# mwhitehill/Tacotron-2

Hardware: AMD Instinct MI355X
Metric: mel-frames/sec (decoder) + audio-samples/sec (WaveNet) @1/2/4/8 MI355X (higher is better)
Workload: dtype f32; 1 GPU; configs[1]: Tacotron-2 encoder+decoder+Postnet inference, batch=32x200-char synthetic, T_out=1000, 1 batch per GPU; global_batch=32, chars=200, t_out=1000, decoded_steps=1000, ref_frames=400, parallelism=utterance-batch sharding x1

## Files before the change

tacotron-2_amd/csrc/common.h:

```cpp
#pragma once
#include <hip/hip_runtime.h>

#include <cstdint>
#include <cstdio>
#include <cstdlib>
#include <map>
#include <stdexcept>
#include <string>
#include <vector>

#include "../../include/tt2.h"

namespace tt2 {

struct Error : std::runtime_error {
  int status;
  Error(int s, const std::string& m) : std::runtime_error(m), status(s) {}
};

void set_last_error(const std::string& msg);

#define TT2_HIP(call)                                                                      \
  do {                                                                                     \
    hipError_t e_ = (call);                                                                \
// ... 102 lines not shown

void put_tensor(WeightMap& wm, const char* name, const float* host, const int64_t* shape, int ndim);
const HostTensor& need(const WeightMap& wm, const std::string& name, std::vector<int64_t> shape);

typedef float f32x4 __attribute__((ext_vector_type(4)));

__host__ __device__ inline int af_idx(int m, int k) {
  const int s = k >> 2, kk = k & 3, h = m >> 4, i = m & 15;
  return ((((s >> 2) * 2 + h) * 64 + (kk * 16 + i)) << 2) + (s & 3);
}
__host__ __device__ inline int wf_idx(int k, int j) {
  const int s = k >> 2, kk = k & 3;
  return ((((s >> 2) * 64) + (kk * 16 + j)) << 2) + (s & 3);
}

constexpr float KG_SB = 1024.f, KG_UNSCALE = 1.f / 1024.f, KG_BMAX = 63.9f;
typedef _Float16 kg_f16x4 __attribute__((ext_vector_type(4)));
typedef unsigned u32x4 __attribute__((ext_vector_type(4)));
__host__ __device__ inline void kg_split1(float v, _Float16& h, _Float16& l) {
  h = (_Float16)v;
  l = (_Float16)(v - (float)h);
}
__host__ __device__ inline void kg_split(const f32x4& v, kg_f16x4& h, kg_f16x4& l) {
#pragma unroll
  for (int e = 0; e < 4; ++e) {
    _Float16 x, y;
    kg_split1(v[e], x, y);
    h[e] = x;
    l[e] = y;
  }
}
struct alignas(16) kg_pk {
  kg_f16x4 h, l;
};
__host__ __device__ inline kg_pk kg_pack(const f32x4& v) {
  kg_pk p;
  kg_split(v, p.h, p.l);
  return p;
}
__host__ __device__ inline kg_pk kg_pk_bits(const u32x4& w) { return __builtin_bit_cast(kg_pk, w); }
__host__ __device__ inline u32x4 kg_bits(const kg_pk& p) { return __builtin_bit_cast(u32x4, p); }
__device__ __forceinline__ kg_pk kg_ld(const float* base, int i4) {
  return kg_pk_bits(reinterpret_cast<const u32x4*>(base)[i4]);
}
__device__ __forceinline__ void kg_mfma_x3_pre(const kg_pk& a0, const kg_pk& a1, const kg_pk& bw, f32x4& c0,
                                               f32x4& c1) {
  c0 = __builtin_amdgcn_mfma_f32_16x16x16f16(a0.l, bw.h, c0, 0, 0, 0);
  c1 = __builtin_amdgcn_mfma_f32_16x16x16f16(a1.l, bw.h, c1, 0, 0, 0);
  c0 = __builtin_amdgcn_mfma_f32_16x16x16f16(a0.h, bw.l, c0, 0, 0, 0);
  c1 = __builtin_amdgcn_mfma_f32_16x16x16f16(a1.h, bw.l, c1, 0, 0, 0);
  c0 = __builtin_amdgcn_mfma_f32_16x16x16f16(a0.h, bw.h, c0, 0, 0, 0);
  c1 = __builtin_amdgcn_mfma_f32_16x16x16f16(a1.h, bw.h, c1, 0, 0, 0);
}
__device__ __forceinline__ void kg_mfma_x3(const f32x4& a0, const f32x4& a1, const f32x4& bw, f32x4& c0,
                                           f32x4& c1) {
  kg_f16x4 a0h, a0l, a1h, a1l, bh, bl;
  kg_split(a0, a0h, a0l);
  kg_split(a1, a1h, a1l);
  kg_split(bw, bh, bl);
  c0 = __builtin_amdgcn_mfma_f32_16x16x16f16(a0l, bh, c0, 0, 0, 0);
  c1 = __builtin_amdgcn_mfma_f32_16x16x16f16(a1l, bh, c1, 0, 0, 0);
  c0 = __builtin_amdgcn_mfma_f32_16x16x16f16(a0h, bl, c0, 0, 0, 0);
  c1 = __builtin_amdgcn_mfma_f32_16x16x16f16(a1h, bl, c1, 0, 0, 0);
  c0 = __builtin_amdgcn_mfma_f32_16x16x16f16(a0h, bh, c0, 0, 0, 0);
  c1 = __builtin_amdgcn_mfma_f32_16x16x16f16(a1h, bh, c1, 0, 0, 0);
}

__device__ __forceinline__ void skinny_mfma(const float* __restrict__ X, const float* __restrict__ Wt,
                                            int sg0, int sg1, f32x4& acc0, f32x4& acc1, int lane) {
  const f32x4* Xv = reinterpret_cast<const f32x4*>(X);
  const f32x4* Wv = reinterpret_cast<const f32x4*>(Wt);
#pragma unroll 4
  for (int sg = sg0; sg < sg1; ++sg) {
    const f32x4 a0 = Xv[(sg * 2 + 0) * 64 + lane];
    const f32x4 a1 = Xv[(sg * 2 + 1) * 64 + lane];
    const f32x4 b = Wv[sg * 64 + lane];
#pragma unroll
    for (int j = 0; j < 4; ++j) {
      acc0 = __builtin_amdgcn_mfma_f32_16x16x4f32(a0[j], b[j], acc0, 0, 0, 0);
      acc1 = __builtin_amdgcn_mfma_f32_16x16x4f32(a1[j], b[j], acc1, 0, 0, 0);
    }
  }
}

template <int NPW>
__device__ __forceinline__ void skinny_mfma_all(const float* __restrict__ X, const float* __restrict__ Wt,
                                                int sg0, f32x4& acc0, f32x4& acc1, int lane) {
  const f32x4* Xv = reinterpret_cast<const f32x4*>(X);
  const f32x4* Wv = reinterpret_cast<const f32x4*>(Wt);
  f32x4 a0[NPW], a1[NPW], b[NPW];
#pragma unroll
  for (int j = 0; j < NPW; ++j) {
    b[j] = Wv[(sg0 + j) * 64 + lane];
    a0[j] = Xv[((sg0 + j) * 2 + 0) * 64 + lane];
    a1[j] = Xv[((sg0 + j) * 2 + 1) * 64 + lane];
  }
  __builtin_amdgcn_sched_barrier(0);
#pragma unroll
  for (int j = 0; j < NPW; ++j)
#pragma unroll
    for (int e = 0; e < 4; ++e) {
      acc0 = __builtin_amdgcn_mfma_f32_16x16x4f32(a0[j][e], b[j][e], acc0, 0, 0, 0);
      acc1 = __builtin_amdgcn_mfma_f32_16x16x4f32(a1[j][e], b[j][e], acc1, 0, 0, 0);
    }
}

// ... 131 lines not shown
```

tacotron-2_amd/csrc/decode_persist.hip:

```cpp
#include "decode_persist.h"

namespace tt2 {

typedef unsigned u32x2 __attribute__((ext_vector_type(2)));

typedef __attribute__((address_space(1))) float pd_gf32;
typedef __attribute__((address_space(1))) unsigned pd_gu32;
typedef __attribute__((address_space(1))) int pd_gi32;
typedef __attribute__((address_space(1))) unsigned long long pd_gu64;
#define PD_RLX __ATOMIC_RELAXED, __HIP_MEMORY_SCOPE_AGENT

#ifndef PD_TAG_H1
#define PD_TAG_H1 0
#endif
constexpr long long PD_TIMEOUT = 200000000LL;
constexpr int PD_LDS_FLOATS = 16384 * 2 + 4096 + 512 * 5 + 288 + 256 * 2 + 32 + 16 + 16 + 16 + 512;

__device__ __forceinline__ float pd_ld(const float* p) {
  return __hip_atomic_load((pd_gf32*)const_cast<float*>(p), PD_RLX);
}
__device__ __forceinline__ void pd_st(float* p, float v) { __hip_atomic_store((pd_gf32*)p, v, PD_RLX); }
__device__ __forceinline__ u32x4 pd_ld4(const float* base, int i4) {
  const auto r = __builtin_amdgcn_make_buffer_rsrc(const_cast<float*>(base), (short)0, 0x7fffffff, 0x00020000);
  return __builtin_amdgcn_raw_buffer_load_b128(r, i4 * 16, 0, 16);
}
__device__ __forceinline__ f32x4 pd_ld4f(const float* base, int i4) { return __builtin_bit_cast(f32x4, pd_ld4(base, i4)); }
__device__ __forceinline__ u32x2 pd_ld2(const float* base, int i2) {
  const auto r = __builtin_amdgcn_make_buffer_rsrc(const_cast<float*>(base), (short)0, 0x7fffffff, 0x00020000);
  return __builtin_amdgcn_raw_buffer_load_b64(r, i2 * 8, 0, 16);
}

template <class F>
__device__ __forceinline__ bool pd_spin(const PdArgs& a, int ph, int lane, F cond) {
  long long t0 = 0;
  for (unsigned spin = 0;; ++spin) {
    if (__all(cond())) return true;
    if ((spin & 63) == 0) {
      const long long now = __builtin_amdgcn_s_memrealtime();
      if (spin == 0) {
        t0 = now;
      } else if (__hip_atomic_load((pd_gi32*)(a.ctl + 2), PD_RLX) != 0 || now - t0 > PD_TIMEOUT) {
        if (lane == 0) __hip_atomic_store((pd_gi32*)(a.ctl + 2), 1 + ph, PD_RLX);
        return false;
      }
    }
    for (int z = 0; z < a.poll_sleep; ++z) __builtin_amdgcn_s_sleep(1);
  }
}

__device__ __forceinline__ unsigned pd_flag(const unsigned* f) {
  return __hip_atomic_load((pd_gu32*)const_cast<unsigned*>(f), PD_RLX);
}

__device__ __forceinline__ bool pd_poll(const PdArgs& a, int ph, int base, int stride, int n, unsigned need, int shift,
                                        int lane) {
  const unsigned* f = a.flags + ph * PD_NB + base;
  return pd_spin(a, ph, lane, [&] { return lane >= n || (pd_flag(f + lane * stride) >> shift) >= need; });
}

__device__ __forceinline__ bool pd_poll_all(const PdArgs& a, int ph, int nprod, unsigned need, int shift, int lane,
                                            bool sweep_first) {
  const int g = blockIdx.x, x = g >> 3, s = g & 7;
  const unsigned* f = a.flags + ph * PD_NB + 32 * s;
  unsigned* f2 = a.flags2 + ph * PD_NB + 8 * x;
  if (sweep_first) {
    const unsigned* fa = a.flags + ph * PD_NB;
    bool ok = true;
#pragma unroll
    for (int i = 0; i < 4; ++i) {
      const int pidx = lane + 64 * i;
      ok = ok && (pidx >= nprod || (pd_flag(fa + pidx) >> shift) >= need);
    }
    if (__all(ok)) {
      if (lane == 0) __hip_atomic_store((pd_gu32*)(f2 + s), need, PD_RLX);
      return true;
    }
  }
  if (!pd_spin(a, ph, lane, [&] { return lane >= 32 || 32 * s + lane >= nprod || (pd_flag(f + lane) >> shift) >= need; }))
    return false;
  if (lane == 0) __hip_atomic_store((pd_gu32*)(f2 + s), need, PD_RLX);
  return pd_spin(a, ph, lane, [&] { return lane >= 8 || pd_flag(f2 + lane) >= need; });
}

__device__ __forceinline__ bool pd_poll_rep(const PdArgs& a, int ph, int r, int base, unsigned need, int lane,
                                            int n = 32) {
  const unsigned* f = a.rflags + (r * PD_NREP + (blockIdx.x & (PD_NREP - 1))) * PD_NB + base;
  return pd_spin(a, ph, lane, [&] { return lane >= n || pd_flag(f + lane) >= need; });
}

template <class F>
__device__ __forceinline__ bool pd_block_wait(int* slot, F poll) {
  if (threadIdx.x < 64) {
    const bool ok = poll();
    if (threadIdx.x == 0) *slot = ok;
  }
  __syncthreads();
  return *slot != 0;
}

__device__ __forceinline__ void pd_putw(unsigned long long* g, unsigned tag, unsigned w) {
  __hip_atomic_store((pd_gu64*)g, ((unsigned long long)tag << 32) | w, PD_RLX);
}
// ... 118 lines not shown

__device__ __forceinline__ void pd_hint(const PdArgs& a, int ph, unsigned val, int tid) {
  __syncthreads();
  if (tid == 0) __hip_atomic_store((pd_gu32*)(a.flags + ph * PD_NB + blockIdx.x), val, PD_RLX);
}
__device__ __forceinline__ void pd_hint_rep(const PdArgs& a, int r, unsigned val, int tid) {
  __syncthreads();
  if (tid < PD_NREP) __hip_atomic_store((pd_gu32*)(a.rflags + (r * PD_NREP + tid) * PD_NB + blockIdx.x), val, PD_RLX);
}

__device__ __forceinline__ void pd_publish_rep(const PdArgs& a, int r, unsigned val, int tid) {
  asm volatile("s_waitcnt vmcnt(0)" ::: "memory");
  __syncthreads();
  if (tid < PD_NREP) __hip_atomic_store((pd_gu32*)(a.rflags + (r * PD_NREP + tid) * PD_NB + blockIdx.x), val, PD_RLX);
}

__device__ __forceinline__ void put_partials(const f32x4& acc0, const f32x4& acc1, float* red, int w, int lane) {
#pragma unroll
  for (int r = 0; r < 4; ++r) {
    const int n = lane & 15, m = (lane >> 4) * 4 + r;
    red[w * 512 + m * 16 + n] = acc0[r];
    red[w * 512 + (m + 16) * 16 + n] = acc1[r];
  }
}
template <int NW>
__device__ __forceinline__ float sum_partials(const float* red, int idx) {
  float v = red[idx];
#pragma unroll
  for (int ww = 1; ww < NW; ++ww) v += red[ww * 512 + idx];
  return v;
}

__device__ __forceinline__ void tail_bar(int* ctr, unsigned& gen, int lane) {
  gen += 4;
  asm volatile("s_waitcnt lgkmcnt(0)" ::: "memory");
  if (lane == 0) __hip_atomic_fetch_add(ctr, 1, __ATOMIC_RELEASE, __HIP_MEMORY_SCOPE_WORKGROUP);
  while ((unsigned)__hip_atomic_load(ctr, __ATOMIC_ACQUIRE, __HIP_MEMORY_SCOPE_WORKGROUP) < gen)
    __builtin_amdgcn_s_sleep(0);
}

#define PD_STAMP(i)                                                                   \
  do {                                                                                \
    if (stp && tid == 0) stp[g * 32 + (i)] = __builtin_amdgcn_s_memrealtime();        \
  } while (0)

template <bool EMT, int TM, bool FL>
__global__ __launch_bounds__(PD_NT) void k_decode_persist(PdArgs a) {
  static_assert(TM == PD_TMAX || (TM == PD_TMAX_LONG && !EMT), "k_decode_persist geometry");
  static_assert(!FL || (!EMT && TM == PD_TMAX), "floor instance: the Tacotron decoder only");
  const auto mm = [](const u32x4& x0, const u32x4& x1, const kg_pk& bw, f32x4& c0, f32x4& c1) {
    if constexpr (FL) asm volatile("" ::"v"(x0), "v"(x1), "v"(kg_bits(bw)));
    else kg_mfma_x3_pre(pd_unx(x0), pd_unx(x1), bw, c0, c1);
  };
  const auto mmo = [](const u32x4& x0, const u32x4& x1, const kg_pk& bw, f32x4& c0, f32x4& c1) {
    if constexpr (FL) asm volatile("" ::"v"(x0), "v"(x1), "v"(kg_bits(bw)));
    else kg_mfma_x3_pre(kg_pk_bits(x0), kg_pk_bits(x1), bw, c0, c1);
  };
  const auto mmg = [](const u32x4& g0, const u32x4& g1, const kg_pk& bw, f32x4& c0, f32x4& c1) {
    if constexpr (FL) asm volatile("" ::"v"(g0), "v"(g1), "v"(kg_bits(bw)));
    else kg_mfma_x3_pre(pd_ung(g0), pd_ung(g1), bw, c0, c1);
  };
  const auto mmf = [](const f32x4& a0, const f32x4& a1, const kg_pk& bw, f32x4& c0, f32x4& c1) {
    kg_mfma_x3_pre(kg_pack(a0), kg_pack(a1), bw, c0, c1);
  };
  constexpr int NI = TM / 128;
  constexpr int NWE = TM / 64;
  constexpr int CWN = TM == PD_TMAX ? 288 : 544;
  extern __shared__ __attribute__((aligned(16))) float sm[];
  float* const sW1h = sm;
  float* const sW2h = sm + 16384;
  float* const red = sm + 32768;
  float* const G = red + 4096;
  float* const RG1 = G + 512;
  float* const RG2 = RG1 + 512;
  float* const RGc = RG2 + 512;
  float* const PPh = RGc + 512;
  float* const cw = PPh + 512;
  float* const al = TM == PD_TMAX ? cw + 288 : red + 2048;
  float* const x1 = cw + 544;
  float* const ssa = x1 + 256;
  float* const qv = ssa + 32;
  float* const sc = qv + 16;
  int* const si = reinterpret_cast<int*>(sc + 16);
  const int g = blockIdx.x, tid_ = threadIdx.x;
  const int b = (g & 7) * 4 + ((g >> 3) & 3), j = g >> 5;
  const bool rowv = b < a.B;
  constexpr int NTL = EMT ? PD_NTILE + PD_ENT : PD_NTILE;
  const bool isproj = g < NTL * PD_KSP;
  const int pn = g % NTL, pks = g / NTL;
  const bool isq = EMT && isproj && pn >= PD_NTILE;
  const int K1S = EMT ? a.K1 : PD_P + PD_E2;
  const int T = a.T_in;
  const int sib0 = (b >> 2) + 8 * (b & 3);
  long long* const stp0 = a.stamps;

  const int tid = tid_, lane = tid & 63, w = tid >> 6;
  const int em = (tid >> 2) & 31, eu = tid & 3;
  kg_pk w1p[2], w2i[8];
  {
    const float* L1 = a.l1_w + (long)g * K1S * 16;
    const float* L2 = a.l2_w + (long)g * PD_H * 16;
#pragma unroll
    for (int i = 0; i < 2; ++i) w1p[i] = kg_ld(L1, (2 * w + i) * 64 + lane);
#pragma unroll
    for (int i = 0; i < 8; ++i) w2i[i] = kg_ld(L2, (8 * w + i) * 64 + lane);
    const f32x4* L1h = reinterpret_cast<const f32x4*>(a.l1_wh + (long)g * PD_H * 16);
    const f32x4* L2h = reinterpret_cast<const f32x4*>(a.l2_wh + (long)g * PD_H * 16);
    f32x4* d1 = reinterpret_cast<f32x4*>(sW1h);
    f32x4* d2 = reinterpret_cast<f32x4*>(sW2h);
    for (int e = tid; e < PD_H * 4; e += PD_NT) {
      d1[e] = L1h[e];
      d2[e] = L2h[e];
    }
  }
  const f32x4 zero4 = {0.f, 0.f, 0.f, 0.f};
  const kg_pk zeropk = kg_pk_bits(u32x4{0u, 0u, 0u, 0u});
  kg_pk wpc = zeropk;
  if (isproj && w < 4 && !isq) wpc = kg_ld(a.proj_w + (long)pn * (PD_H + PD_E2) * 16, (PD_H / 16 + 4 * pks + w) * 64 + lane);
  const float* const WPH = a.proj_w + (long)pn * (PD_H + PD_E2) * 16 + (8 * pks) * 64 * 4;
  kg_pk w1c[4];
  {
    const float* W1C = a.l1_w + (long)g * K1S * 16 + (PD_P / 16 + 4 * w) * 64 * 4;
#pragma unroll
    for (int i = 0; i < 4; ++i) w1c[i] = kg_ld(W1C, i * 64 + lane);
  }
  kg_pk w1e = zeropk, wdf = zeropk;
  if constexpr (EMT) {
    if (w < a.e_XW / 16)
      w1e = kg_ld(a.l1_w + (long)g * K1S * 16, ((PD_P + PD_E2) / 16 + w) * 64 + lane);
    if (a.e_dense && isq && w < a.e_KC / 128)
      wdf = kg_ld(a.e_wd + (long)(pn - PD_NTILE) * a.e_KC * 16, (pks * (a.e_KC / 128) + w) * 64 + lane);
  }
  f32x4* const swl = reinterpret_cast<f32x4*>(si + 16);
  if (tid < 128) swl[tid] = reinterpret_cast<const f32x4*>(a.loc_cw + (long)j * PD_KLP * 16)[tid];
  float* const cst = RG1;
  const int u0 = pd_unit(g, 0);
  if (tid < 128) {
#pragma unroll
    for (int q = 0; q < 4; ++q) {
      const int u = pd_unit(g, eu);
      const int col = (u >> 2) * 16 + 4 * q + (u & 3);
      cst[q * 128 + tid] = a.l1_b[col] + (EMT && a.e_spk1 ? a.e_spk1[(long)em * 4 * PD_H + col] : 0.f);
      cst[(4 + q) * 128 + tid] = a.l2_b[col];
      cst[(8 + q) * 128 + tid] = a.GS[(long)em * 4 * PD_H + col];
    }
  }
  float c1 = 0.f, c2 = 0.f;
  const int len = rowv ? a.lengths[b] : 0;
  const float va_k = a.va[16 * j + (lane & 15)];
  const float b2p = a.pre_b2[32 * j + (tid & 31)];
  for (int e = tid; e < CWN; e += PD_NT) cw[e] = 0.f;
  if (tid < TM) al[tid] = 0.f;
  if (tid < 32) ssa[tid] = 0.f;
  if (tid == 0) {
    si[0] = 0;
    si[4] = 0;
    si[8] = 0;
    sc[2] = 0.f;
  }
  f32x4 vals[8];
  {
    const f32x4* V = reinterpret_cast<const f32x4*>(a.valuesT + ((long)(rowv ? b : 0) * PD_E2 + 64 * j + (tid & 63)) * TM +
                                                    32 * (tid >> 6));
#pragma unroll
    for (int i = 0; i < 8; ++i) vals[i] = V[i];
  }
  f32x4 loc[NI];
#pragma unroll
  for (int i = 0; i < NI; ++i) loc[i] = zero4;
  f32x4 accC0 = zero4, accC1 = zero4;
  if constexpr (EMT) {
    const float* XE = a.EMTx + 32 * PD_EQ;
    mmf(pd_ld4f(XE, (w * 2) * 64 + lane), pd_ld4f(XE, (w * 2 + 1) * 64 + lane), w1e, accC0, accC1);
  }
  f32x4 q1a = zero4, q1b = zero4, q2a = zero4, q2b = zero4;
  const long BP = (long)a.B * PD_P;

// ... 13 lines not shown
  auto prenet_ops = [&](float k1, float k2, int tid) {
    PrenetOps o;
    o.keep1 = k1;
    o.keep2 = k2;
    const f32x4* W2 = reinterpret_cast<const f32x4*>(a.pre_w2t + (long)(32 * j + (tid & 31)) * PD_P + 16 * (tid >> 5));
#pragma unroll
    for (int i = 0; i < 4; ++i) o.w2p[i] = W2[i];
    return o;
  };
  auto prenet = [&](const PrenetOps& o, auto pre1, int par, unsigned tag, int tid) {
    if (tid >= 256) {
      const int pos = tid - 256;
      const int col = 16 * (pos >> 4) + ((pos >> 2) & 3) + 4 * (pos & 3);
      x1[col] = rowv ? (fmaxf(pre1(pos), 0.f) / 0.5f) * o.keep1 : 0.f;
      if (pos < 32) red[3072 + pos] = o.keep2;
    }
    __syncthreads();
    {
      const int k16 = tid >> 5;
      float s = 0.f;
#pragma unroll
      for (int i = 0; i < 16; ++i)
        if (!FL || i == 0) s += x1[16 * k16 + i] * o.w2p[i >> 2][i & 3];
      s += __shfl_xor(s, 32);
      if ((tid & 63) < 32) red[(tid >> 6) * 32 + (tid & 31)] = s;
    }
    __syncthreads();
    if (tid < 32) {
      float v = 0.f;
#pragma unroll
      for (int ww = 0; ww < 8; ++ww) v += red[ww * 32 + tid];
      const int n = 32 * j + tid;
      const float out = rowv ? (fmaxf(v + b2p, 0.f) / 0.5f) * red[3072 + tid] : 0.f;
      pd_putw(a.PREg + par * 32 * PD_P + af_idx(b, n), tag, pd_split1(out));
    }
  };

  auto rec_half = [&](int ph, const float* X, unsigned tb, const float* Wl, int h, f32x4& Qa, f32x4& Qb, int w,
                      int lane, bool check, bool pin) {
    u32x4 xv[8];
    const auto ix = [&](int i) { return ((8 * w + 4 * h + (i >> 1)) * 2 + (i & 1)) * 64 + lane; };
    if (check) {
      if (!pd_take4<8>(a, ph, X, ix, tb, xv, [] { return true; })) si[8] = 1;
    } else {
#pragma unroll
      for (int i = 0; i < 8; ++i) xv[i] = pd_ld4(X, ix(i));
      if (pin) __builtin_amdgcn_sched_barrier(0);
    }
    if (h == 0) {
      Qa = a.zo * Qa;
      Qb = a.zo * Qb;
    }
#pragma unroll
    for (int i = 0; i < 4; ++i) {
      const int sg = 8 * w + 4 * h + i;
      if (!PD_TAG_H1 && ph == PD_F_H1) mmo(xv[2 * i], xv[2 * i + 1], kg_ld(Wl, sg * 64 + lane), Qa, Qb);
      else mm(xv[2 * i], xv[2 * i + 1], kg_ld(Wl, sg * 64 + lane), Qa, Qb);
    }
  };
  __syncthreads();
  {
    float k1, k2;
    prenet_keep(0, tid, k1, k2);
    prenet(prenet_ops(k1, k2, tid), [&](int pos) { return a.pre_b1[pos]; }, 0, 1u << 1, tid);
  }
  if (tid == 0) si[1] = 0;
  __syncthreads();

  for (int t = 0; t < a.max_iters; ++t) {
    const unsigned tg = t + 1;
    const int p = t & 1;
    const unsigned tb = pd_tb(t), tbp = pd_tb(t - 1);
    long long* const stp = (stp0 && t == a.stamp_step) ? stp0 : nullptr;
    int tid = tid_, lane, w, em, eu;
    asm volatile("" : "+v"(tid));
    lane = tid & 63;
    w = tid >> 6;
    em = (tid >> 2) & 31;
    eu = tid & 3;
    PD_STAMP(0);
    if constexpr (!EMT) {
      if (stp && tid == 0) stp[g * 32 + 31] = __builtin_amdgcn_s_getreg(0x1814) & 15;
    }
    float keep1n, keep2n;
    prenet_keep(t + 1, tid, keep1n, keep2n);
    u32x4 a0[2], a1[2];
    {
      const auto rp = __builtin_amdgcn_make_buffer_rsrc(a.PREg + p * 32 * PD_P, (short)0, 0x7fffffff, 0x00020000);
      unsigned sb[2] = {0u, 0u};
      long long t0 = 0;
      for (unsigned spin = 0;; ++spin) {
        bool ok = true;
#pragma unroll
        for (int i = 0; i < 2; ++i)
#pragma unroll
          for (int h = 0; h < 2; ++h) {
            const int fo = (((2 * w + i) * 2 + h) * 64 + lane) * 4;
            const auto q0 = __builtin_amdgcn_raw_buffer_load_b128(rp, fo * 8, 0, 16);
            const auto q1 = __builtin_amdgcn_raw_buffer_load_b128(rp, fo * 8 + 16, 0, 16);
            const u32x4 v = {q0[0], q0[2], q1[0], q1[2]};
            ok = ok && (q0[1] >> 1) == tg && (q0[3] >> 1) == tg && (q1[1] >> 1) == tg && (q1[3] >> 1) == tg;
            if (h == 0) a0[i] = v;
            else a1[i] = v;
            if (i == 0) sb[h] = q0[1] & 1u;
          }
        if (__all(ok)) break;
        if ((spin & 31) == 0) {
          const long long now = __builtin_amdgcn_s_memrealtime();
          if (spin == 0) {
            t0 = now;
          } else if (__hip_atomic_load((pd_gi32*)(a.ctl + 2), PD_RLX) != 0 || now - t0 > PD_TIMEOUT) {
            if (lane == 0) {
              __hip_atomic_store((pd_gi32*)(a.ctl + 2), 1 + PD_F_PRE, PD_RLX);
              atomicMax(si + 1, 2);
            }
            break;
          }
        }
        for (int z = 0; z < a.poll_sleep; ++z) __builtin_amdgcn_s_sleep(1);
      }
      if (t > 0 && w == 0) {
        int dn;
        if (a.T_lim > 0) {
          dn = t >= a.T_lim;
        } else {
          const int r0 = lane & 15;
          const bool v0 = lane < 16 && r0 < a.B, v1 = lane < 16 && r0 + 16 < a.B;
          const unsigned long long f0 = __ballot(v0 && sb[0]), f1 = __ballot(v1 && sb[1]);
          const unsigned long long m0 = __ballot(v0), m1 = __ballot(v1);
          dn = a.stop_at_any == 2 ? 0 : (f0 == m0 && f1 == m1);
        }
        if (lane == 0 && dn) atomicMax(si + 1, 1);
      }
    }
    PD_STAMP(1);
    {
      f32x4 s0 = accC0 + a.one_m_zo * q1a, s1 = accC1 + a.one_m_zo * q1b;
#pragma unroll
      for (int i = 0; i < 2; ++i) mmg(a0[i], a1[i], w1p[i], s0, s1);
      PD_STAMP(18);
      put_partials(s0, s1, red, w, lane);
      __syncthreads();
      PD_STAMP(19);
    }
    if (si[1]) {
      if (si[1] == 1 && g == 0 && tid == 0) {
        a.ctl[1] = t;
        a.ctl[0] = 1;
      }
      return;
    }
    if (tid < 128) {
      float z[4];
#pragma unroll
      for (int q = 0; q < 4; ++q) {
        const int idx = em * 16 + 4 * q + eu;
        z[q] = (sum_partials<8>(red, idx) * KG_UNSCALE + ssa[em] * cst[(8 + q) * 128 + tid]) + cst[q * 128 + tid];
      }
      const float cn = sigm_fast(z[2] + 1.0f) * c1 + sigm_fast(z[0]) * tanh_rcp(z[1]);
      const float hn = sigm_fast(z[3]) * tanh_rcp(cn);
      c1 = a.one_m_zo * cn + a.zo * c1;
      pd_st_h4(a.H1x + p * 32 * PD_H, em, u0, hn, lane, PD_TAG_H1 ? tb : ~0u);
    }
    if constexpr (PD_TAG_H1) pd_hint_rep(a, 0, tg, tid);
    else pd_publish_rep(a, 0, tg, tid);
    PD_STAMP(2);
    if (t > 0) rec_half(PD_F_H2, a.H2x + (p ^ 1) * 32 * PD_H, tbp, sW2h, 1, q2a, q2b, w, lane, false, true);
    PD_STAMP(3);
    if constexpr (!PD_TAG_H1)
      if (!pd_poll_rep(a, PD_F_H1, 0, 32 * w, tg, lane)) si[8] = 1;
    PD_STAMP(4);
    {
      const float* X = a.H1x + p * 32 * PD_H;
      f32x4 s0 = a.one_m_zo * q2a, s1 = a.one_m_zo * q2b;
#pragma unroll
      for (int h = 0; h < 2; ++h) {
        u32x4 xv[8];
        const auto ix = [&](int i) { return ((8 * w + 4 * h + (i >> 1)) * 2 + (i & 1)) * 64 + lane; };
        if constexpr (PD_TAG_H1 == 0) {
#pragma unroll
          for (int i = 0; i < 8; ++i) xv[i] = pd_ld4(X, ix(i));
          __builtin_amdgcn_sched_barrier(0);
        } else if constexpr (PD_TAG_H1 == 1) {
          if (!pd_take4<8>(a, PD_F_H1, X, ix, tb, xv, [&] { return pd_poll_rep(a, PD_F_H1, 0, 32 * w, tg, lane); }))
            si[8] = 1;
        } else {
          if (!pd_take4<8>(a, PD_F_H1, X, ix, tb, xv, [] { return true; })) si[8] = 1;
        }
#pragma unroll
        for (int i = 0; i < 4; ++i) {
          if constexpr (PD_TAG_H1) mm(xv[2 * i], xv[2 * i + 1], w2i[4 * h + i], s0, s1);
          else mmo(xv[2 * i], xv[2 * i + 1], w2i[4 * h + i], s0, s1);
        }
      }
      PD_STAMP(16);
      put_partials(s0, s1, red, w, lane);
      __syncthreads();
      PD_STAMP(17);
      if (si[8]) return;
    }
    if (tid < 128) {
      float z[4];
#pragma unroll
      for (int q = 0; q < 4; ++q) {
        const int idx = em * 16 + 4 * q + eu;
        z[q] = sum_partials<8>(red, idx) * KG_UNSCALE + cst[(4 + q) * 128 + tid];
      }
      const float cn = sigm_fast(z[2] + 1.0f) * c2 + sigm_fast(z[0]) * tanh_rcp(z[1]);
      const float hn = sigm_fast(z[3]) * tanh_rcp(cn);
      c2 = a.one_m_zo * cn + a.zo * c2;
      pd_st_h4(a.H2x + p * 32 * PD_H, em, u0, hn, lane, tb);
    }
    pd_hint_rep(a, 1, tg, tid);
    PD_STAMP(5);
    f32x4 wq[8];
    {
      const f32x4* Q = reinterpret_cast<const f32x4*>(a.q_wt + (long)(16 * j + (tid & 15)) * PD_H + 32 * (tid >> 4));
#pragma unroll
      for (int i = 0; i < 8; ++i) wq[i] = Q[i];
    }
    f32x4 kv[NI];
    {
      const f32x4* K = reinterpret_cast<const f32x4*>(a.keysT + ((long)(rowv ? b : 0) * PD_A + 16 * j + (lane & 15)) * TM);
#pragma unroll
      for (int i = 0; i < NI; ++i) kv[i] = K[(w + 8 * i) * 4 + (lane >> 4)];
    }
    rec_half(PD_F_H1, a.H1x + p * 32 * PD_H, tb, sW1h, 0, q1a, q1b, w, lane, false, false);
    PD_STAMP(6);
    PD_STAMP(7);

    if (rowv) {
      const float* X = a.H2x + p * 32 * PD_H;
      u32x2 hg[2];
      if (!pd_takev<2>(a, PD_F_H2, X, [&](int i) { return af_idx(b, 128 * w + 64 * i + lane) >> 1; }, tb, hg,
                       [&] { return pd_poll_rep(a, PD_F_H2, 1, 32 * w, tg, lane); }))
        si[8] = 1;
      red[128 * w + lane] = FL ? __uint_as_float(hg[0][0]) : pd_val(hg[0], (lane >> 2) & 1);
      red[128 * w + 64 + lane] = FL ? __uint_as_float(hg[1][0]) : pd_val(hg[1], (lane >> 2) & 1);
      __builtin_amdgcn_wave_barrier();
      {
        const int seg = tid >> 4;
        float s = 0.f;
        if constexpr (FL) {
          s = red[seg * 32];
          asm volatile("" ::"v"(wq[0]), "v"(wq[1]), "v"(wq[2]), "v"(wq[3]), "v"(wq[4]), "v"(wq[5]), "v"(wq[6]), "v"(wq[7]));
        } else {
#pragma unroll
          for (int ii = 0; ii < 32; ++ii) s += red[seg * 32 + ii] * wq[ii >> 2][ii & 3];
          s += __shfl_xor(s, 16);
          s += __shfl_xor(s, 32);
        }
        if (lane < 16) red[1024 + w * 16 + lane] = s;
      }
      __syncthreads();
      float qk = 0.f;
#pragma unroll
      for (int ww = 0; ww < 8; ++ww) qk += red[1024 + ww * 16 + (lane & 15)];
      unsigned long long* E = a.Eg + (((long)p * 32 + b) * 8 + j) * TM;
      float sel[NI];
#pragma unroll
      for (int i = 0; i < NI; ++i) {
        float e4[4];
#pragma unroll
        for (int r = 0; r < 4; ++r)
          e4[r] = FL ? kv[i][r] + qk + loc[i][r] : sum16(va_k * tanh_rcp(kv[i][r] + qk + loc[i][r]));
        const int rr = lane & 3;
        sel[i] = rr == 0 ? e4[0] : rr == 1 ? e4[1] : rr == 2 ? e4[2] : e4[3];
      }
      const int src = ((lane >> 2) & 3) * 16 + (lane & 3);
      float vi[NI];
#pragma unroll
      for (int i = 0; i < NI; ++i) vi[i] = __shfl(sel[i], src);
      float vo = vi[0];
#pragma unroll
      for (int i = 1; i < NI; ++i) vo = (lane >> 4) == i ? vi[i] : vo;
      if (lane < 16 * NI) pd_put(E + (w + 8 * (lane >> 4)) * 16 + (lane & 15), tg, vo);
    }
    __syncthreads();
    if (si[8]) return;
    PD_STAMP(8);
    if (isproj) {
      const float* X = a.H2x + p * 32 * PD_H;
      const int sg = 8 * pks + w;
      f32x4 s0 = zero4, s1 = zero4;
      u32x4 xv[2];
      if (!pd_take4<2>(a, PD_F_H2, X, [&](int i) { return (sg * 2 + i) * 64 + lane; }, tb, xv,
                       [&] { return pd_poll_rep(a, PD_F_H2, 1, 32 * pks, tg, lane); }))
        si[8] = 1;
      mm(xv[0], xv[1], kg_ld(WPH, w * 64 + lane), s0, s1);
      reduce_waves_32x16<8>(s0, s1, red, G, w, lane, tid);
      if (isq) {
        const int m = tid >> 4, col = tid & 15;
        pd_put(a.QEg + (((long)p * PD_KSP + pks) * 32 + m) * PD_EQ + 16 * (pn - PD_NTILE) + col, tg, G[tid]);
      } else {
        PPh[tid] = G[tid];
      }
    }
    PD_STAMP(9);
    if (rowv) {
      const unsigned long long* E = a.Eg + ((long)p * 32 + b) * 8 * TM;
      f32x4 vhi[TM == PD_TMAX ? 1 : 8];
      if constexpr (TM != PD_TMAX) {
        const f32x4* V = reinterpret_cast<const f32x4*>(a.valuesT + ((long)(rowv ? b : 0) * PD_E2 + 64 * j + (tid & 63)) * TM +
                                                        PD_TMAX + 32 * (tid >> 6));
#pragma unroll
        for (int i = 0; i < 8; ++i) vhi[i] = V[i];
      }
      if (tid == 0) si[5] = 1;
      __syncthreads();
      float e = -INFINITY;
      if (tid < TM) {
        float ev[8];
        if (!pd_take<8>(a, PD_F_E, E, tid, TM, tg, tid < T, ev)) si[5] = 0;
        if (tid < T) {
          e = 0.f;
#pragma unroll
          for (int jj = 0; jj < 8; ++jj) e += ev[jj];
          if (a.constraint) {
            const int pm = si[0], wn = a.win;
            bool masked;
            if (a.monotonic) masked = (tid < pm) || (tid >= pm + wn);
            else masked = (tid < pm - (wn / 2 + (wn % 2 != 0 ? 1 : 0))) || (tid >= pm + wn / 2);
            if (masked) e = -4294967296.0f;
          }
          if (a.mask_encoder && tid >= len) e = -INFINITY;
        }
        const float mx = wave_max_dpp(e);
        if (lane == 0) red[w] = mx;
      }
      __syncthreads();
      if (!si[5]) return;
      float ex = 0.f;
      if (tid < TM) {
        float mx = fmaxf(fmaxf(red[0], red[1]), fmaxf(red[2], red[3]));
        if constexpr (NWE == 8) mx = fmaxf(mx, fmaxf(fmaxf(red[4], red[5]), fmaxf(red[6], red[7])));
        ex = tid < T ? __expf(e - mx) : 0.f;
        const float sum = wave_sum_dpp(ex);
        if (lane == 0) red[8 + w] = sum;
      }
      __syncthreads();
      PD_STAMP(21);
      if (tid < TM) {
        float den = (red[8] + red[9]) + (red[10] + red[11]);
        if constexpr (NWE == 8) den += (red[12] + red[13]) + (red[14] + red[15]);
        al[tid] = tid < T ? ex * __builtin_amdgcn_rcpf(den) : 0.f;
      }
      __syncthreads();
      if (tid < T) {
        const float cp = cw[15 + tid];
        cw[15 + tid] = a.cumulative ? al[tid] + cp : al[tid];
        if (j == 0 && a.align) a.align[((long)b * a.max_iters + t) * T + tid] = al[tid];
      }
      if (w == 1) {
        float best = -INFINITY, ss = 0.f;
        int bi = 0x7fffffff;
        for (int i = lane; i < T; i += 64) {
          if (al[i] > best) {
            best = al[i];
            bi = i;
          }
          if (i < len) ss += al[i];
        }
        for (int o = 32; o > 0; o >>= 1) {
          const float ob = __shfl_xor(best, o);
          const int oi = __shfl_xor(bi, o);
          if (ob > best || (ob == best && oi < bi)) {
            best = ob;
            bi = oi;
          }
          ss += __shfl_xor(ss, o);
        }
        if (lane == 0) {
          si[0] = bi;
          sc[2] = ss;
        }
      }
      {
        const int c = tid & 63, ts = tid >> 6;
        float s = 0.f;
#pragma unroll
        for (int i = 0; i < 32; ++i)
          if (!FL || i == 0) s += al[ts * 32 + i] * vals[i >> 2][i & 3];
        if constexpr (FL) asm volatile("" ::"v"(vals[1]), "v"(vals[2]), "v"(vals[3]), "v"(vals[4]), "v"(vals[5]), "v"(vals[6]), "v"(vals[7]));
        if constexpr (TM != PD_TMAX) {
#pragma unroll
          for (int i = 0; i < 32; ++i) s += al[PD_TMAX + ts * 32 + i] * vhi[i >> 2][i & 3];
        }
        red[ts * 64 + c] = s;
      }
      __syncthreads();
      if (tid < 64) {
        float s = 0.f;
#pragma unroll
        for (int ts = 0; ts < 8; ++ts) s += red[ts * 64 + tid];
        const int src = tid & ~12;
        const f32x4 v = {__shfl(s, src), __shfl(s, src + 4), __shfl(s, src + 8), __shfl(s, src + 12)};
        if ((tid & 12) == 0) pd_st_x4(a.CTXx + p * 32 * PD_E2, af_idx(b, 64 * j + tid) >> 2, v, tb);
      }
      if (tid == 64 && j == 0) pd_st(a.SSx + p * 32 + b, pd_tag(sc[2], tb));
    } else {
      if (tid < 64 && (tid & 12) == 0) pd_st_x4(a.CTXx + p * 32 * PD_E2, af_idx(b, 64 * j + tid) >> 2, zero4, tb);
      if (tid == 64 && j == 0) pd_st(a.SSx + p * 32 + b, pd_tag(0.f, tb));
    }
    if constexpr (EMT) {
      if (tid == 0) si[6] = 1;
    }
    pd_hint(a, PD_F_CTX, tg, tid);
    PD_STAMP(10);
    rec_half(PD_F_H1, a.H1x + p * 32 * PD_H, tb, sW1h, 1, q1a, q1b, w, lane, false, true);
#pragma unroll
    for (int i = 0; i < NI; ++i) {
      const int t0 = (w + 8 * i) * 16 + (lane & 15) + (lane >> 4);
      f32x4 l = zero4;
#pragma unroll
      for (int sg = 0; sg < 2; ++sg)
#pragma unroll
        for (int e = 0; e < 4; ++e)
          if constexpr (FL) asm volatile("" ::"v"(cw[t0 + 16 * sg + 4 * e]), "v"(swl[64 * sg + lane][e]));
          else l = __builtin_amdgcn_mfma_f32_16x16x4f32(cw[t0 + 16 * sg + 4 * e], swl[64 * sg + lane][e], l, 0, 0, 0);
      loc[i] = l;
    }
    if constexpr (EMT) {
      if (g >= PD_EG0) {
        const int r0 = 2 * (g - PD_EG0);
        float* qe = red;
        float* sco = red + 256;
        float* vls = red + 256 + 2 * a.e_heads * a.e_Tv;
        const int nv = a.e_Tv * a.e_Dv;
        const bool vl = 256 + 2 * a.e_heads * a.e_Tv + 2 * nv <= 4096;
        float vt[8];
#pragma unroll
        for (int u = 0; u < 8; ++u) {
          const int e = tid + PD_NT * u, rr = e >= nv, b2 = r0 + rr;
          vt[u] = (vl && e < 2 * nv && b2 < a.B) ? a.e_val[b2 * a.e_vbs + (e - rr * nv)] : 0.f;
        }
        {
          const int row = r0 + ((tid >> 7) & 1), col = tid & 127, hs = tid >> 8;
          float pv[PD_KSP / 2];
          if (!pd_take<PD_KSP / 2>(a, PD_F_QE, a.QEg + (((long)p * PD_KSP + 4 * hs) * 32 + row) * PD_EQ, col, 32 * PD_EQ,
                                   tg, true, pv))
            si[6] = 0;
          G[tid] = (pv[0] + pv[1]) + (pv[2] + pv[3]);
        }
        if (vl)
#pragma unroll
          for (int u = 0; u < 8; ++u)
            if (tid + PD_NT * u < 2 * nv) vls[tid + PD_NT * u] = vt[u];
        __syncthreads();
        if (tid < 256) qe[tid] = (G[tid] + G[256 + tid]) * KG_UNSCALE + a.e_qrow[(r0 + (tid >> 7)) * PD_EQ + (tid & 127)];
        __syncthreads();
        PD_STAMP(22);
        if (!si[6]) return;
// ... 164 lines not shown
        prenet(pops, [&](int pos) { return tp[pos]; }, p ^ 1, ((tg + 1) << 1) | (unsigned)stopbit, tid);
      } else {
        prenet(pops, [&](int pos) { return red[PD_NPJ + pos]; }, p ^ 1, ((tg + 1) << 1) | (unsigned)stopbit, tid);
      }
    }
    __syncthreads();
    PD_STAMP(14);
#ifdef PD_XSTAMP
    if constexpr (!EMT) {
      if (stp) {
        asm volatile("s_waitcnt vmcnt(0)" ::: "memory");
        PD_STAMP(30);
      }
    }
#endif
    if constexpr (EMT) {
      if (g >= PD_EG0 && a.e_dense) {
        const int r0 = 2 * (g - PD_EG0);
        {
          const int row = r0 + ((tid >> 7) & 1), col = tid & 127, hs = tid >> 8;
          float pv[PD_KSP / 2];
          if (!pd_take<PD_KSP / 2>(a, PD_F_EO, a.EOg + (((long)p * PD_KSP + 4 * hs) * 32 + row) * PD_EQ, col, 32 * PD_EQ,
                                   tg, true, pv))
            si[6] = 0;
          G[tid] = (pv[0] + pv[1]) + (pv[2] + pv[3]);
        }
        __syncthreads();
        if (tid < 256) {
          const int row = r0 + (tid >> 7), col = tid & 127;
          float o = (G[tid] + G[256 + tid]) * KG_UNSCALE + a.e_bd[col];
          if (a.e_spk && row < a.B) o += a.e_spk[row * PD_EQ + col];
          pd_st(a.EMTx + p * 32 * PD_EQ + af_idx(row, col), row < a.B ? o : 0.f);
        }
        PD_STAMP(27);
        pd_publish_rep(a, 2, tg, tid);
        PD_STAMP(28);
        if (!si[6]) return;
      }
    }
    {
      const float* XC = a.CTXx + p * 32 * PD_E2;
      accC0 = zero4;
      accC1 = zero4;
      u32x4 xv[8];
      if (!pd_take4<8>(a, PD_F_CTX, XC, [&](int i) { return ((4 * w + (i >> 1)) * 2 + (i & 1)) * 64 + lane; }, tb, xv,
                       [&] {
                         if constexpr (!EMT) {
                           if (stp && lane == 0) stp[g * 32 + 22 + w] = __builtin_amdgcn_s_memrealtime();
                         }
                         return pd_poll(a, PD_F_CTX, 32 * w, 1, 32, tg, 0, lane);
                       }))
        si[8] = 1;
#pragma unroll
      for (int i = 0; i < 4; ++i) mm(xv[2 * i], xv[2 * i + 1], w1c[i], accC0, accC1);
      if (w == 0) {
        float sv[1];
        if (!pd_take1<1>(a, PD_F_CTX, a.SSx + p * 32, [&](int) { return lane & 31; }, tb, sv,
                         [&] { return pd_poll(a, PD_F_CTX, 0, 1, 32, tg, 0, lane); }))
          si[8] = 1;
        if (lane < 32) ssa[lane] = sv[0];
      }
    }
    if constexpr (EMT) {
      if (!pd_block_wait(si + 6, [&] { return pd_poll_rep(a, PD_F_EMT, 2, PD_EG0, tg, lane, 16); })) return;
      PD_STAMP(29);
      const float* XE = a.EMTx + p * 32 * PD_EQ;
      mmf(pd_ld4f(XE, (w * 2) * 64 + lane), pd_ld4f(XE, (w * 2 + 1) * 64 + lane), w1e, accC0, accC1);
    }
    PD_STAMP(15);
  }
  if (g == 0 && tid == 0) {
    a.ctl[1] = a.max_iters;
    a.ctl[0] = 1;
  }
}

size_t pd_lds_bytes() { return sizeof(float) * (size_t)PD_LDS_FLOATS; }

bool pd_device_ok(int dev) {
  hipDeviceProp_t prop;
  if (hipGetDeviceProperties(&prop, dev) != hipSuccess) return false;
  if (prop.multiProcessorCount < PD_NB) return false;
  for (const void* k : {reinterpret_cast<const void*>(k_decode_persist<false, PD_TMAX, false>),
                        reinterpret_cast<const void*>(k_decode_persist<true, PD_TMAX, false>),
                        reinterpret_cast<const void*>(k_decode_persist<false, PD_TMAX_LONG, false>),
                        reinterpret_cast<const void*>(k_decode_persist<false, PD_TMAX, true>)})
    if (hipFuncSetAttribute(k, hipFuncAttributeMaxDynamicSharedMemorySize, (int)pd_lds_bytes()) != hipSuccess)
      return false;
  int nb = 0, ne = 0, nl = 0;
  if (hipOccupancyMaxActiveBlocksPerMultiprocessor(&nb, k_decode_persist<false, PD_TMAX, false>, PD_NT, pd_lds_bytes()) != hipSuccess ||
      hipOccupancyMaxActiveBlocksPerMultiprocessor(&ne, k_decode_persist<true, PD_TMAX, false>, PD_NT, pd_lds_bytes()) != hipSuccess ||
      hipOccupancyMaxActiveBlocksPerMultiprocessor(&nl, k_decode_persist<false, PD_TMAX_LONG, false>, PD_NT, pd_lds_bytes()) !=
          hipSuccess)
    return false;
  return nb >= 1 && ne >= 1 && nl >= 1;
}

void pd_launch(const PdArgs& a, hipStream_t s, bool emt, int tm) {
  TT2_CHECK(tm == PD_TMAX || (tm == PD_TMAX_LONG && !emt), TT2_ERR_INVALID_ARG, "persistent decoder: unsupported geometry");
  TT2_CHECK(a.T_in >= 1 && a.T_in <= tm, TT2_ERR_INVALID_ARG, "persistent decoder: T_in outside the kernel's range");
  PdArgs arg = a;
  void* params[] = {&arg};
  static const bool floor_env = env_on("TT2_PD_FLOOR", false);
  const void* k = emt ? reinterpret_cast<const void*>(k_decode_persist<true, PD_TMAX, false>)
                  : tm != PD_TMAX ? reinterpret_cast<const void*>(k_decode_persist<false, PD_TMAX_LONG, false>)
                  : floor_env     ? reinterpret_cast<const void*>(k_decode_persist<false, PD_TMAX, true>)
                                  : reinterpret_cast<const void*>(k_decode_persist<false, PD_TMAX, false>);
// ... 5 lines not shown
```

Measured before the change: 1.271 million mel-frames/s.

## Use 16x16x32 f16 MFMA, prefetch projection input, parallelize alignment argmax/sum

Pairs adjacent K-slices into 8-wide f16 operands so the split-precision (hi/lo) GEMMs in the persistent decoder issue half as many MFMAs, using the 16x16x32 f16 instruction. The LDS weight copy is re-laid out to match the paired format. Other changes: the H2 input for the projection is loaded early with a tag check to skip a poll, one __syncthreads is dropped, and the serial single-wave argmax/sum over the alignment is replaced by per-wave DPP reductions merged by one thread. This cuts instruction count and latency on the per-step critical path, but the pairing must match the 16x16x32 operand K ordering or results will be wrong.

```diff
diff --git a/tacotron-2_amd/csrc/common.h b/tacotron-2_amd/csrc/common.h
--- a/tacotron-2_amd/csrc/common.h
+++ b/tacotron-2_amd/csrc/common.h
@@ -178,6 +178,32 @@
   c0 = __builtin_amdgcn_mfma_f32_16x16x16f16(a0.h, bw.h, c0, 0, 0, 0);
   c1 = __builtin_amdgcn_mfma_f32_16x16x16f16(a1.h, bw.h, c1, 0, 0, 0);
 }
+typedef _Float16 kg_f16x8 __attribute__((ext_vector_type(8)));
+struct alignas(16) kg_pk2 {
+  kg_f16x8 h, l;
+};
+__device__ __forceinline__ kg_pk2 kg_pair(const kg_pk& p, const kg_pk& q) {
+  kg_pk2 r;
+  r.h = __builtin_shufflevector(p.h, q.h, 0, 1, 2, 3, 4, 5, 6, 7);
+  r.l = __builtin_shufflevector(p.l, q.l, 0, 1, 2, 3, 4, 5, 6, 7);
+  return r;
+}
+__device__ __forceinline__ kg_pk2 kg_ld2(const float* base, int pr, int lane) {
+  const u32x4* v = reinterpret_cast<const u32x4*>(base);
+  kg_pk2 r;
+  r.h = __builtin_bit_cast(kg_f16x8, v[(pr * 2 + 0) * 64 + lane]);
+  r.l = __builtin_bit_cast(kg_f16x8, v[(pr * 2 + 1) * 64 + lane]);
+  return r;
+}
+__device__ __forceinline__ void kg_mfma_x3_pre2(const kg_pk2& a0, const kg_pk2& a1, const kg_pk2& bw, f32x4& c0,
+                                                f32x4& c1) {
+  c0 = __builtin_amdgcn_mfma_f32_16x16x32_f16(a0.l, bw.h, c0, 0, 0, 0);
+  c1 = __builtin_amdgcn_mfma_f32_16x16x32_f16(a1.l, bw.h, c1, 0, 0, 0);
+  c0 = __builtin_amdgcn_mfma_f32_16x16x32_f16(a0.h, bw.l, c0, 0, 0, 0);
+  c1 = __builtin_amdgcn_mfma_f32_16x16x32_f16(a1.h, bw.l, c1, 0, 0, 0);
+  c0 = __builtin_amdgcn_mfma_f32_16x16x32_f16(a0.h, bw.h, c0, 0, 0, 0);
+  c1 = __builtin_amdgcn_mfma_f32_16x16x32_f16(a1.h, bw.h, c1, 0, 0, 0);
+}
 __device__ __forceinline__ void kg_mfma_x3(const f32x4& a0, const f32x4& a1, const f32x4& bw, f32x4& c0,
                                            f32x4& c1) {
   kg_f16x4 a0h, a0l, a1h, a1l, bh, bl;
diff --git a/tacotron-2_amd/csrc/decode_persist.hip b/tacotron-2_amd/csrc/decode_persist.hip
--- a/tacotron-2_amd/csrc/decode_persist.hip
+++ b/tacotron-2_amd/csrc/decode_persist.hip
@@ -48,6 +48,16 @@
   }
 }
 
+__device__ __forceinline__ int pd_wave_min(int v) {
+  v = min(v, dpp_i<DPP_XOR1>(v));
+  v = min(v, dpp_i<DPP_XOR2>(v));
+  v = min(v, dpp_i<DPP_HALF_MIRROR>(v));
+  v = min(v, dpp_i<DPP_MIRROR>(v));
+  v = min(v, __builtin_amdgcn_update_dpp(v, v, 0x142, 0xA, 0xF, false));
+  v = min(v, __builtin_amdgcn_update_dpp(v, v, 0x143, 0xC, 0xF, false));
+  return __builtin_amdgcn_readlane(v, 63);
+}
+
 __device__ __forceinline__ unsigned pd_flag(const unsigned* f) {
   return __hip_atomic_load((pd_gu32*)const_cast<unsigned*>(f), PD_RLX);
 }
@@ -272,16 +282,27 @@
     if constexpr (FL) asm volatile("" ::"v"(x0), "v"(x1), "v"(kg_bits(bw)));
     else kg_mfma_x3_pre(pd_unx(x0), pd_unx(x1), bw, c0, c1);
   };
-  const auto mmo = [](const u32x4& x0, const u32x4& x1, const kg_pk& bw, f32x4& c0, f32x4& c1) {
-    if constexpr (FL) asm volatile("" ::"v"(x0), "v"(x1), "v"(kg_bits(bw)));
-    else kg_mfma_x3_pre(kg_pk_bits(x0), kg_pk_bits(x1), bw, c0, c1);
-  };
-  const auto mmg = [](const u32x4& g0, const u32x4& g1, const kg_pk& bw, f32x4& c0, f32x4& c1) {
-    if constexpr (FL) asm volatile("" ::"v"(g0), "v"(g1), "v"(kg_bits(bw)));
-    else kg_mfma_x3_pre(pd_ung(g0), pd_ung(g1), bw, c0, c1);
-  };
   const auto mmf = [](const f32x4& a0, const f32x4& a1, const kg_pk& bw, f32x4& c0, f32x4& c1) {
     kg_mfma_x3_pre(kg_pack(a0), kg_pack(a1), bw, c0, c1);
+  };
+  const auto sink2 = [](const u32x4& p0, const u32x4& p1, const u32x4& q0, const u32x4& q1, const kg_pk2& bw) {
+    asm volatile("" ::"v"(p0), "v"(p1), "v"(q0), "v"(q1), "v"(__builtin_bit_cast(u32x4, bw.h)),
+                 "v"(__builtin_bit_cast(u32x4, bw.l)));
+  };
+  const auto mm2 = [&](const u32x4& p0, const u32x4& p1, const u32x4& q0, const u32x4& q1, const kg_pk2& bw, f32x4& c0,
+                       f32x4& c1) {
+    if constexpr (FL) sink2(p0, p1, q0, q1, bw);
+    else kg_mfma_x3_pre2(kg_pair(pd_unx(p0), pd_unx(q0)), kg_pair(pd_unx(p1), pd_unx(q1)), bw, c0, c1);
+  };
+  const auto mmo2 = [&](const u32x4& p0, const u32x4& p1, const u32x4& q0, const u32x4& q1, const kg_pk2& bw, f32x4& c0,
+                        f32x4& c1) {
+    if constexpr (FL) sink2(p0, p1, q0, q1, bw);
+    else kg_mfma_x3_pre2(kg_pair(kg_pk_bits(p0), kg_pk_bits(q0)), kg_pair(kg_pk_bits(p1), kg_pk_bits(q1)), bw, c0, c1);
+  };
+  const auto mmg2 = [&](const u32x4& p0, const u32x4& p1, const u32x4& q0, const u32x4& q1, const kg_pk2& bw, f32x4& c0,
+                        f32x4& c1) {
+    if constexpr (FL) sink2(p0, p1, q0, q1, bw);
+    else kg_mfma_x3_pre2(kg_pair(pd_ung(p0), pd_ung(q0)), kg_pair(pd_ung(p1), pd_ung(q1)), bw, c0, c1);
   };
   constexpr int NI = TM / 128;
   constexpr int NWE = TM / 64;
@@ -316,21 +337,25 @@
 
   const int tid = tid_, lane = tid & 63, w = tid >> 6;
   const int em = (tid >> 2) & 31, eu = tid & 3;
-  kg_pk w1p[2], w2i[8];
+  kg_pk2 w1p, w2i[4];
   {
     const float* L1 = a.l1_w + (long)g * K1S * 16;
     const float* L2 = a.l2_w + (long)g * PD_H * 16;
-#pragma unroll
-    for (int i = 0; i < 2; ++i) w1p[i] = kg_ld(L1, (2 * w + i) * 64 + lane);
-#pragma unroll
-    for (int i = 0; i < 8; ++i) w2i[i] = kg_ld(L2, (8 * w + i) * 64 + lane);
-    const f32x4* L1h = reinterpret_cast<const f32x4*>(a.l1_wh + (long)g * PD_H * 16);
-    const f32x4* L2h = reinterpret_cast<const f32x4*>(a.l2_wh + (long)g * PD_H * 16);
-    f32x4* d1 = reinterpret_cast<f32x4*>(sW1h);
-    f32x4* d2 = reinterpret_cast<f32x4*>(sW2h);
+    w1p = kg_pair(kg_ld(L1, (2 * w) * 64 + lane), kg_ld(L1, (2 * w + 1) * 64 + lane));
+#pragma unroll
+    for (int i = 0; i < 4; ++i) w2i[i] = kg_pair(kg_ld(L2, (8 * w + 2 * i) * 64 + lane), kg_ld(L2, (8 * w + 2 * i + 1) * 64 + lane));
+    const u32x4* L1h = reinterpret_cast<const u32x4*>(a.l1_wh + (long)g * PD_H * 16);
+    const u32x4* L2h = reinterpret_cast<const u32x4*>(a.l2_wh + (long)g * PD_H * 16);
+    u32x2* d1 = reinterpret_cast<u32x2*>(sW1h);
+    u32x2* d2 = reinterpret_cast<u32x2*>(sW2h);
     for (int e = tid; e < PD_H * 4; e += PD_NT) {
-      d1[e] = L1h[e];
-      d2[e] = L2h[e];
+      const int sg = e >> 6, l = e & 63;
+      const int dh = (((sg >> 1) * 2 + 0) * 64 + l) * 2 + (sg & 1), dl = (((sg >> 1) * 2 + 1) * 64 + l) * 2 + (sg & 1);
+      const u32x4 v1 = L1h[e], v2 = L2h[e];
+      d1[dh] = u32x2{v1[0], v1[1]};
+      d1[dl] = u32x2{v1[2], v1[3]};
+      d2[dh] = u32x2{v2[0], v2[1]};
+      d2[dl] = u32x2{v2[2], v2[3]};
     }
   }
   const f32x4 zero4 = {0.f, 0.f, 0.f, 0.f};
@@ -338,11 +363,11 @@
   kg_pk wpc = zeropk;
   if (isproj && w < 4 && !isq) wpc = kg_ld(a.proj_w + (long)pn * (PD_H + PD_E2) * 16, (PD_H / 16 + 4 * pks + w) * 64 + lane);
   const float* const WPH = a.proj_w + (long)pn * (PD_H + PD_E2) * 16 + (8 * pks) * 64 * 4;
-  kg_pk w1c[4];
+  kg_pk2 w1c[2];
   {
     const float* W1C = a.l1_w + (long)g * K1S * 16 + (PD_P / 16 + 4 * w) * 64 * 4;
 #pragma unroll
-    for (int i = 0; i < 4; ++i) w1c[i] = kg_ld(W1C, i * 64 + lane);
+    for (int i = 0; i < 2; ++i) w1c[i] = kg_pair(kg_ld(W1C, (2 * i) * 64 + lane), kg_ld(W1C, (2 * i + 1) * 64 + lane));
   }
   kg_pk w1e = zeropk, wdf = zeropk;
   if constexpr (EMT) {
@@ -462,10 +487,10 @@
       Qb = a.zo * Qb;
     }
 #pragma unroll
-    for (int i = 0; i < 4; ++i) {
-      const int sg = 8 * w + 4 * h + i;
-      if (!PD_TAG_H1 && ph == PD_F_H1) mmo(xv[2 * i], xv[2 * i + 1], kg_ld(Wl, sg * 64 + lane), Qa, Qb);
-      else mm(xv[2 * i], xv[2 * i + 1], kg_ld(Wl, sg * 64 + lane), Qa, Qb);
+    for (int i = 0; i < 2; ++i) {
+      const kg_pk2 bw = kg_ld2(Wl, 4 * w + 2 * h + i, lane);
+      if (!PD_TAG_H1 && ph == PD_F_H1) mmo2(xv[4 * i], xv[4 * i + 1], xv[4 * i + 2], xv[4 * i + 3], bw, Qa, Qb);
+      else mm2(xv[4 * i], xv[4 * i + 1], xv[4 * i + 2], xv[4 * i + 3], bw, Qa, Qb);
     }
   };
   __syncthreads();
@@ -546,8 +571,7 @@
     PD_STAMP(1);
     {
       f32x4 s0 = accC0 + a.one_m_zo * q1a, s1 = accC1 + a.one_m_zo * q1b;
-#pragma unroll
-      for (int i = 0; i < 2; ++i) mmg(a0[i], a1[i], w1p[i], s0, s1);
+      mmg2(a0[0], a1[0], a0[1], a1[1], w1p, s0, s1);
       PD_STAMP(18);
       put_partials(s0, s1, red, w, lane);
       __syncthreads();
@@ -598,9 +622,9 @@
           if (!pd_take4<8>(a, PD_F_H1, X, ix, tb, xv, [] { return true; })) si[8] = 1;
         }
 #pragma unroll
-        for (int i = 0; i < 4; ++i) {
-          if constexpr (PD_TAG_H1) mm(xv[2 * i], xv[2 * i + 1], w2i[4 * h + i], s0, s1);
-          else mmo(xv[2 * i], xv[2 * i + 1], w2i[4 * h + i], s0, s1);
+        for (int i = 0; i < 2; ++i) {
+          if constexpr (PD_TAG_H1) mm2(xv[4 * i], xv[4 * i + 1], xv[4 * i + 2], xv[4 * i + 3], w2i[2 * h + i], s0, s1);
+          else mmo2(xv[4 * i], xv[4 * i + 1], xv[4 * i + 2], xv[4 * i + 3], w2i[2 * h + i], s0, s1);
         }
       }
       PD_STAMP(16);
@@ -638,7 +662,11 @@
     rec_half(PD_F_H1, a.H1x + p * 32 * PD_H, tb, sW1h, 0, q1a, q1b, w, lane, false, false);
     PD_STAMP(6);
     PD_STAMP(7);
-
+    u32x4 xph[2];
+    const auto projh_ld = [&] {
+#pragma unroll
+      for (int i = 0; i < 2; ++i) xph[i] = pd_ld4(a.H2x + p * 32 * PD_H, ((8 * pks + w) * 2 + i) * 64 + lane);
+    };
     if (rowv) {
       const float* X = a.H2x + p * 32 * PD_H;
       u32x2 hg[2];
@@ -663,6 +691,7 @@
         if (lane < 16) red[1024 + w * 16 + lane] = s;
       }
       __syncthreads();
+      if (isproj) projh_ld();
       float qk = 0.f;
 #pragma unroll
       for (int ww = 0; ww < 8; ++ww) qk += red[1024 + ww * 16 + (lane & 15)];
@@ -686,6 +715,7 @@
       for (int i = 1; i < NI; ++i) vo = (lane >> 4) == i ? vi[i] : vo;
       if (lane < 16 * NI) pd_put(E + (w + 8 * (lane >> 4)) * 16 + (lane & 15), tg, vo);
     }
+    if (tid == 0) si[5] = 1;
     __syncthreads();
     if (si[8]) return;
     PD_STAMP(8);
@@ -693,11 +723,12 @@
       const float* X = a.H2x + p * 32 * PD_H;
       const int sg = 8 * pks + w;
       f32x4 s0 = zero4, s1 = zero4;
-      u32x4 xv[2];
-      if (!pd_take4<2>(a, PD_F_H2, X, [&](int i) { return (sg * 2 + i) * 64 + lane; }, tb, xv,
+      const bool hit = rowv && __all(pd_ok4(xph[0], tb) && pd_ok4(xph[1], tb));
+      if (!hit &&
+          !pd_take4<2>(a, PD_F_H2, X, [&](int i) { return (sg * 2 + i) * 64 + lane; }, tb, xph,
                        [&] { return pd_poll_rep(a, PD_F_H2, 1, 32 * pks, tg, lane); }))
         si[8] = 1;
-      mm(xv[0], xv[1], kg_ld(WPH, w * 64 + lane), s0, s1);
+      mm(xph[0], xph[1], kg_ld(WPH, w * 64 + lane), s0, s1);
       reduce_waves_32x16<8>(s0, s1, red, G, w, lane, tid);
       if (isq) {
         const int m = tid >> 4, col = tid & 15;
@@ -716,8 +747,6 @@
 #pragma unroll
         for (int i = 0; i < 8; ++i) vhi[i] = V[i];
       }
-      if (tid == 0) si[5] = 1;
-      __syncthreads();
       float e = -INFINITY;
       if (tid < TM) {
         float ev[8];
@@ -753,7 +782,16 @@
       if (tid < TM) {
         float den = (red[8] + red[9]) + (red[10] + red[11]);
         if constexpr (NWE == 8) den += (red[12] + red[13]) + (red[14] + red[15]);
-        al[tid] = tid < T ? ex * __builtin_amdgcn_rcpf(den) : 0.f;
+        const float av = tid < T ? ex * __builtin_amdgcn_rcpf(den) : 0.f;
+        al[tid] = av;
+        const float wm = wave_max_dpp(av);
+        const int wi = pd_wave_min(tid < T && av == wm ? tid : 0x7fffffff);
+        const float ws = wave_sum_dpp(tid < len ? av : 0.f);
+        if (lane == 0) {
+          G[w] = wm;
+          G[8 + w] = __int_as_float(wi);
+          G[16 + w] = ws;
+        }
       }
       __syncthreads();
       if (tid < T) {
@@ -761,30 +799,6 @@
         cw[15 + tid] = a.cumulative ? al[tid] + cp : al[tid];
         if (j == 0 && a.align) a.align[((long)b * a.max_iters + t) * T + tid] = al[tid];
       }
-      if (w == 1) {
-        float best = -INFINITY, ss = 0.f;
-        int bi = 0x7fffffff;
-        for (int i = lane; i < T; i += 64) {
-          if (al[i] > best) {
-            best = al[i];
-            bi = i;
-          }
-          if (i < len) ss += al[i];
-        }
-        for (int o = 32; o > 0; o >>= 1) {
-          const float ob = __shfl_xor(best, o);
-          const int oi = __shfl_xor(bi, o);
-          if (ob > best || (ob == best && oi < bi)) {
-            best = ob;
-            bi = oi;
-          }
-          ss += __shfl_xor(ss, o);
-        }
-        if (lane == 0) {
-          si[0] = bi;
-          sc[2] = ss;
-        }
-      }
       {
         const int c = tid & 63, ts = tid >> 6;
         float s = 0.f;
@@ -807,7 +821,21 @@
         const f32x4 v = {__shfl(s, src), __shfl(s, src + 4), __shfl(s, src + 8), __shfl(s, src + 12)};
         if ((tid & 12) == 0) pd_st_x4(a.CTXx + p * 32 * PD_E2, af_idx(b, 64 * j + tid) >> 2, v, tb);
       }
-      if (tid == 64 && j == 0) pd_st(a.SSx + p * 32 + b, pd_tag(sc[2], tb));
+      if (tid == 64) {
+        float best = G[0], ss = G[16];
+        int bi = __float_as_int(G[8]);
+#pragma unroll
+        for (int ww = 1; ww < NWE; ++ww) {
+          if (G[ww] > best) {
+            best = G[ww];
+            bi = __float_as_int(G[8 + ww]);
+          }
+          ss += G[16 + ww];
+        }
+        si[0] = bi;
+        sc[2] = ss;
+        if (j == 0) pd_st(a.SSx + p * 32 + b, pd_tag(ss, tb));
+      }
     } else {
       if (tid < 64 && (tid & 12) == 0) pd_st_x4(a.CTXx + p * 32 * PD_E2, af_idx(b, 64 * j + tid) >> 2, zero4, tb);
       if (tid == 64 && j == 0) pd_st(a.SSx + p * 32 + b, pd_tag(0.f, tb));
@@ -1078,7 +1106,7 @@
                        }))
         si[8] = 1;
 #pragma unroll
-      for (int i = 0; i < 4; ++i) mm(xv[2 * i], xv[2 * i + 1], w1c[i], accC0, accC1);
+      for (int i = 0; i < 2; ++i) mm2(xv[4 * i], xv[4 * i + 1], xv[4 * i + 2], xv[4 * i + 3], w1c[i], accC0, accC1);
       if (w == 0) {
         float sv[1];
         if (!pd_take1<1>(a, PD_F_CTX, a.SSx + p * 32, [&](int) { return lane & 31; }, tb, sv,
```

Result: faster. 1.350 million mel-frames/s, median of 6 (+6.2%).
